# TianyiFranklinWang/MIRROR

Hardware: AMD Instinct MI355X
Metric: SSL samples/sec (slide+RNA pairs) (higher is better)
Workload: dtype bf16; 1 GPU; BASELINE c2: B=16/GPU x [4096 patch tokens x 1024-d] + [2048 genes], D=512, RNA depth 6 / 8 heads, train mode, local-batch InfoNCE; precision_policy=bf16, per_gpu_batch=16, global_batch=16, parallelism=dp1, grad_bucket_dtype=f32, step_launch=hip_graph

## Files before the change

mirror_amd/csrc/nystrom_fused.hip:

```cpp
#include <cstdlib>
#include <cstring>
#include "gemm_kernel.h"

namespace {

constexpr int NM = 256;
constexpr int ND = 64;
constexpr int NP = 72;
constexpr int NT = 256;
constexpr int TR = 128;

typedef __attribute__((address_space(3))) s16x4 lds_s16x4;
typedef short s16x8 __attribute__((ext_vector_type(8)));

__device__ __forceinline__ bf16x8 frag_kc(const bf16_t* img, int row0, int k0, int lane) {
    return *reinterpret_cast<const bf16x8*>(img + (row0 + (lane & 31)) * NP + k0 + 8 * (lane >> 5));
}
__device__ __forceinline__ bf16x8 frag_tr(const bf16_t* img, int col0, int kb, int lane) {
    const int g16 = lane >> 4, i = lane & 15, q = i >> 2, p = i & 3;
    const bf16_t* a0 = img + (kb + 4 * (g16 >> 1) + q) * NP + col0 + 16 * (g16 & 1) + 4 * p;
    s16x4 lo = __builtin_amdgcn_ds_read_tr16_b64_v4i16((lds_s16x4*)a0);
    s16x4 hi = __builtin_amdgcn_ds_read_tr16_b64_v4i16((lds_s16x4*)(a0 + 8 * NP));
    s16x8 v = __builtin_shufflevector(lo, hi, 0, 1, 2, 3, 4, 5, 6, 7);
    return __builtin_bit_cast(bf16x8, v);
}
__device__ __forceinline__ bf16x8 frag_g(const bf16_t* rowptr, int k0, int lane) {
    return *reinterpret_cast<const bf16x8*>(rowptr + k0 + 8 * (lane >> 5));
}
template <int T>
__device__ __forceinline__ bf16x8 pack8(const f32x16& a) {
    bf16x8 r;
#pragma unroll
    for (int j = 0; j < 8; j++) r[j] = (__bf16)a[8 * T + j];
    return r;
}
__device__ __forceinline__ f32x16 zero16() {
    f32x16 z;
#pragma unroll
    for (int r = 0; r < 16; r++) z[r] = 0.f;
    return z;
}
#define MFMA(a, b, c) __builtin_amdgcn_mfma_f32_32x32x16_bf16((a), (b), (c), 0, 0, 0)

constexpr float LOG2E = 1.4426950408889634f, LN2 = 0.6931471805599453f;
typedef float f32x8v __attribute__((ext_vector_type(8)));
typedef float f32x2v __attribute__((ext_vector_type(2)));
__device__ __forceinline__ float vsum16(const f32x16& a) {
    const f32x8v t8 = __builtin_shufflevector(a, a, 0, 1, 2, 3, 4, 5, 6, 7) + __builtin_shufflevector(a, a, 8, 9, 10, 11, 12, 13, 14, 15);
    const f32x4 t4 = __builtin_shufflevector(t8, t8, 0, 1, 2, 3) + __builtin_shufflevector(t8, t8, 4, 5, 6, 7);
    const f32x2v t2 = __builtin_shufflevector(t4, t4, 0, 1) + __builtin_shufflevector(t4, t4, 2, 3);
    return t2[0] + t2[1];
}
__device__ __forceinline__ float vmax16(const f32x16& a) {
    float m0 = fmaxf(fmaxf(a[0], a[1]), a[2]), m1 = fmaxf(fmaxf(a[3], a[4]), a[5]), m2 = fmaxf(fmaxf(a[6], a[7]), a[8]);
    float m3 = fmaxf(fmaxf(a[9], a[10]), a[11]), m4 = fmaxf(fmaxf(a[12], a[13]), a[14]);
    return fmaxf(fmaxf(fmaxf(m0, m1), fmaxf(m2, m3)), fmaxf(m4, a[15]));
}
__device__ __forceinline__ void exp2_16(f32x16& a) {
#pragma unroll
    for (int r = 0; r < 16; r++) a[r] = __builtin_amdgcn_exp2f(a[r]);
}
__device__ __forceinline__ f32x16 fma_splat(const f32x16& a, float m, float b) {
    const f32x2v mm = {m, m}, bb = {b, b};
    f32x16 r;
#pragma unroll
    for (int i = 0; i < 16; i += 2) {
        f32x2v x = {a[i], a[i + 1]};
        x = __builtin_elementwise_fma(x, mm, bb);
        r[i] = x[0];
        r[i + 1] = x[1];
    }
    return r;
}
constexpr float NEG_BIG = -1e30f;
__device__ __forceinline__ f32x16 rowvals16(const float* src, int hl) {
    f32x16 v;
#pragma unroll
    for (int gq = 0; gq < 4; gq++) {
        const f32x4 x = *reinterpret_cast<const f32x4*>(src + 8 * gq + 4 * hl);
        v[4 * gq] = x[0]; v[4 * gq + 1] = x[1]; v[4 * gq + 2] = x[2]; v[4 * gq + 3] = x[3];
    }
    return v;
}

template <int ROWS>
__device__ __forceinline__ void stage_rows(bf16_t* img, const bf16_t* __restrict__ src, long ld, int tid) {
#pragma unroll
    for (int i = 0; i < ROWS * 8 / NT; i++) {
        const int cid = tid + i * NT, r = cid >> 3, c = cid & 7;
        *reinterpret_cast<u32x4*>(img + r * NP + c * 8) = *reinterpret_cast<const u32x4*>(src + (long)r * ld + c * 8);
    }
}
template <int ROWS>
__device__ __forceinline__ void tile_load(u32x4 (&regs)[ROWS * 8 / NT], const bf16_t* __restrict__ src, long ld, int tid) {
#pragma unroll
    for (int i = 0; i < ROWS * 8 / NT; i++) {
        const int cid = tid + i * NT, r = cid >> 3, c = cid & 7;
        regs[i] = *reinterpret_cast<const u32x4*>(src + (long)r * ld + c * 8);
    }
}
template <int ROWS>
__device__ __forceinline__ void tile_store(const u32x4 (&regs)[ROWS * 8 / NT], bf16_t* img, int tid) {
#pragma unroll
    for (int i = 0; i < ROWS * 8 / NT; i++) {
        const int cid = tid + i * NT, r = cid >> 3, c = cid & 7;
// ... 323 lines not shown
    const int pr = tid >> 3, pc = tid & 7;
    u32x4 rq[NCH], rg[NCH], ro[NCH];
    float rl = 0.f;
    auto load_tiles = [&](int t) {
#pragma unroll
        for (int i = 0; i < NCH; i++) {
            const long row = (long)t * TR + pr + 64 * i;
            rq[i] = *reinterpret_cast<const u32x4*>(qb + row * 3 * D + pc * 8);
            rg[i] = *reinterpret_cast<const u32x4*>(gb + row * D + pc * 8);
            ro[i] = *reinterpret_cast<const u32x4*>(ob + row * D + pc * 8);
        }
        if (tid < TR) rl = lse1[(long)bh * g.n_p + (long)t * TR + tid];
    };
    load_tiles(t0);
#pragma unroll 1
    for (int t = t0; t < t1; t++) {
        __syncthreads();
#pragma unroll
        for (int i = 0; i < NCH; i++) {
            const int r = pr + 64 * i;
            *reinterpret_cast<u32x4*>(s_q + r * NP + pc * 8) = rq[i];
            *reinterpret_cast<u32x4*>(s_g + r * NP + pc * 8) = rg[i];
            float d = 0.f;
#pragma unroll
            for (int w = 0; w < 4; w++) {
                d += __uint_as_float(rg[i][w] << 16) * __uint_as_float(ro[i][w] << 16);
                d += __uint_as_float(rg[i][w] & 0xffff0000u) * __uint_as_float(ro[i][w] & 0xffff0000u);
            }
            d += __shfl_xor(d, 1, 64);
            d += __shfl_xor(d, 2, 64);
            d += __shfl_xor(d, 4, 64);
            if (pc == 0) {
                s_del[r] = -d * g.scale;
                delta1[(long)bh * g.n_p + (long)t * TR + r] = d;
            }
        }
        if (tid < TR) {
            s_lse[tid] = -rl * LOG2E;
            s_mr[tid] = masked ? g.mrow[(long)b * g.n_p + (long)t * TR + tid] : 1.f;
        }
        __syncthreads();
        if (t + 1 < t1) load_tiles(t + 1);
#pragma unroll
        for (int i = 0; i < 4; i++) {
            const f32x16 lv = rowvals16(s_lse + 32 * i, hl), dv = rowvals16(s_del + 32 * i, hl);
            f32x16 s = zero16(), dp = zero16();
#pragma unroll
            for (int ks = 0; ks < 4; ks++) {
                s = MFMA(frag_kc(s_q, 32 * i, 16 * ks, lane), klf[ks], s);
                dp = MFMA(frag_kc(s_g, 32 * i, 16 * ks, lane), w2f[ks], dp);
            }
            if (masked) {
                const f32x16 vr = rowvals16(s_mr + 32 * i, hl);
                s = s * g.scale2;
                mask_fill16(s, vr, ml);
                s = s + lv;
                exp2_16(s);
                dp = s * (dp * g.scale + dv);
                mask_zero16(dp, vr, ml);
            } else {
                s = s * g.scale2 + lv;
                exp2_16(s);
                dp = s * (dp * g.scale + dv);
            }
            const bf16x8 p0 = pack8<0>(s), p1 = pack8<1>(s), d0 = pack8<0>(dp), d1 = pack8<1>(dp);
#pragma unroll
            for (int nb = 0; nb < 2; nb++) {
                adw[nb] = MFMA(p0, frag_tr(s_g, 32 * nb, 32 * i, lane), adw[nb]);
                adw[nb] = MFMA(p1, frag_tr(s_g, 32 * nb, 32 * i + 16, lane), adw[nb]);
                adk[nb] = MFMA(d0, frag_tr(s_q, 32 * nb, 32 * i, lane), adk[nb]);
                adk[nb] = MFMA(d1, frag_tr(s_q, 32 * nb, 32 * i + 16, lane), adk[nb]);
            }
        }
    }
    float* dwb = dw2 + (long)bh * NM * ND;
    float* dkb = dlm + (long)b * NM * 2 * D + D + hd * ND;
#pragma unroll
    for (int nb = 0; nb < 2; nb++) {
        atomic_tile(dwb + (long)(32 * wave) * ND + 32 * nb, ND, adw[nb], hl, c);
        atomic_tile(dkb + (long)(32 * wave) * 2 * D + 32 * nb, 2 * D, adk[nb], hl, c);
    }
}

constexpr int A3_PART = NM * (ND + 2);
template <bool MASKED, bool RC = false>
__global__ __launch_bounds__(NT, 2) void nys_a3_fwd_kernel(const bf16_t* __restrict__ qkv, const bf16_t* __restrict__ lm,
                                                        float* __restrict__ av, float* __restrict__ lse3, float* __restrict__ part,
                                                        Geo g, int tiles_per_wg) {
    constexpr int VH = RC ? RC_HALO : 0;
    __shared__ __attribute__((aligned(16))) bf16_t s_k[TR * NP];
    __shared__ __attribute__((aligned(16))) bf16_t s_v_[(TR + 2 * VH) * NP];
    __shared__ __attribute__((aligned(16))) float s_mr[TR];
    bf16_t* const s_v = s_v_ + VH * NP;
    const int tid = threadIdx.x, lane = tid & 63, wave = tid >> 6, c = lane & 31, hl = lane >> 5;
    const int bh = blockIdx.y, b = bh / g.h, hd = bh % g.h, D = g.D;
    const long LD = g.lm_ld;
    const int t0 = blockIdx.x * tiles_per_wg, t1 = min(t0 + tiles_per_wg, g.n_p / TR);
    constexpr bool masked = MASKED;
    float ml[2] = {1.f, 1.f};
    if (masked) { ml[0] = g.mlm[(long)b * NM + 64 * wave + c]; ml[1] = g.mlm[(long)b * NM + 64 * wave + 32 + c]; }
    const bf16_t* qlb = lm + (long)b * NM * LD + hd * ND;
    bf16x8 qlf[2][4];
#pragma unroll
    for (int j = 0; j < 2; j++)
#pragma unroll
        for (int ks = 0; ks < 4; ks++) qlf[j][ks] = frag_g(qlb + (long)(64 * wave + 32 * j + c) * LD, 16 * ks, lane);
    const bf16_t* kb = qkv + (long)b * g.n_p * 3 * D + D + hd * ND;
    const bf16_t* vb = kb + D;
    float mrun[2] = {NEG_BIG, NEG_BIG}, lrun[2] = {0.f, 0.f};
    f32x16 o[2][2];
#pragma unroll
    for (int nb = 0; nb < 2; nb++)
#pragma unroll
        for (int j = 0; j < 2; j++) o[nb][j] = zero16();
    u32x4 rk[TR * 8 / NT], rv[TR * 8 / NT];
    tile_load<TR>(rk, kb + (long)t0 * TR * 3 * D, 3 * D, tid);
    tile_load<TR>(rv, vb + (long)t0 * TR * 3 * D, 3 * D, tid);
    u32x4 rh = {0u, 0u, 0u, 0u};
    const int hq = tid >> 3, hc = tid & 7, hrow = hq < RC_HALO ? hq - RC_HALO : TR + hq - RC_HALO;
    auto halo_load = [&](int t) {
        const long sr = (long)t * TR + hrow;
        rh = (u32x4){0u, 0u, 0u, 0u};
        if (sr >= 0 && sr < g.n_p) rh = *reinterpret_cast<const u32x4*>(vb + sr * 3 * D + hc * 8);
    };
    __shared__ __attribute__((aligned(16))) bf16x8 s_wf_[RC ? 4 * 64 : 1];
    if constexpr (RC) {
        halo_load(t0);
        if (wave == 0) {
            const float* wh = g.rc_w + hd * RC_TAPS;
#pragma unroll
            for (int ks = 0; ks < 4; ks++) {
                bf16x8 wv;
#pragma unroll
                for (int e = 0; e < 8; e++) {
                    const int k = 16 * ks + (e < 4 ? 4 * hl + e : 8 + 4 * hl + (e - 4));
                    const int jt = k - c;
                    const float x = wh[min(max(jt, 0), RC_TAPS - 1)];
                    wv[e] = (__bf16)((jt >= 0 && jt < RC_TAPS) ? x : 0.f);
                }
                s_wf_[ks * 64 + lane] = wv;
            }
        }
    }
#pragma unroll 1
    for (int t = t0; t < t1; t++) {
        __syncthreads();
        tile_store<TR>(rk, s_k, tid);
        tile_store<TR>(rv, s_v, tid);
        if constexpr (RC) *reinterpret_cast<u32x4*>(s_v + hrow * NP + hc * 8) = rh;
        if (tid < TR) s_mr[tid] = masked ? g.mrow[(long)b * g.n_p + (long)t * TR + tid] : 1.f;
        __syncthreads();
        if (t + 1 < t1) {
            tile_load<TR>(rk, kb + (long)(t + 1) * TR * 3 * D, 3 * D, tid);
            tile_load<TR>(rv, vb + (long)(t + 1) * TR * 3 * D, 3 * D, tid);
            if constexpr (RC) halo_load(t + 1);
        }
        if constexpr (RC) {
            bf16_t* orow = g.rc_out + ((long)b * g.n_p + (long)t * TR + 32 * wave + c) * D + hd * ND;
            int opq = 0;
            asm volatile("" : "+v"(opq));
            const bf16x8* s_wf = s_wf_ + opq;
#pragma unroll
            for (int nb = 0; nb < 2; nb++) {
                f32x16 a = zero16();
#pragma unroll
                for (int ks = 0; ks < 4; ks++) a = MFMA(frag_tr(s_v, 32 * nb, 32 * wave - RC_HALO + 16 * ks, lane), s_wf[ks * 64 + lane], a);
// ... 439 lines not shown
}

extern "C" int mh_nys_attn1_fwd(const void* qkv, const void* lm, const void* w2, void* out, float* lse1, const float* mrow,
                                const float* mlm, int B, int h, int n_p, int m, int dh, float scale, int accumulate, int64_t lm_ld, void* o1,
                                mh_stream s) {
    if (int e = check_geo("mh_nys_attn1_fwd", B, h, n_p, m, dh)) return e;
    MH_REQUIRE(lm_ld == 0 || (lm_ld >= 2L * h * ND && lm_ld % 8 == 0), "mh_nys_attn1_fwd: lm_ld must be 0 or a multiple of 8 >= 2 D");
    if (B == 0) return MH_OK;
    MH_REQUIRE((mrow == nullptr) == (mlm == nullptr), "mh_nys_attn1_fwd: mrow and mlm go together");
    const Geo g{h, n_p, h * ND, scale, scale * LOG2E, mrow, mlm, accumulate, lm_ld > 0 ? lm_ld : 2L * h * ND, nullptr, nullptr};
    MH_REQUIRE((((uintptr_t)o1) & 15) == 0, "mh_nys_attn1_fwd: o1 must be 16-byte aligned");
    NYS_LAUNCH(nys_a1_fwd_kernel, dim3(pick_walkers(B * h, n_p), B * h), dim3(NT), 0, (hipStream_t)s, (const bf16_t*)qkv, (const bf16_t*)lm,
                       (const bf16_t*)w2, (bf16_t*)out, lse1, g, Q8Out{}, (bf16_t*)o1);
    MH_LAUNCH_CHECK("mh_nys_attn1_fwd");
    return MH_OK;
}

extern "C" int mh_nys_attn1_fwd_q8(const void* qkv, const void* lm, const void* w2, void* out, float* lse1, int B, int h, int n_p, int m,
                                   int dh, float scale, int accumulate, void* q8, unsigned* ring, const float* tick, float margin,
                                   float* q8_scale, void* o1, mh_stream s) {
    if (int e = check_geo("mh_nys_attn1_fwd_q8", B, h, n_p, m, dh)) return e;
    if (B == 0) return MH_OK;
    MH_REQUIRE(q8 && ring && tick && q8_scale && margin >= 1.f && ((uintptr_t)q8 & 3) == 0, "mh_nys_attn1_fwd_q8: q8, ring, tick, scale and margin >= 1");
    const Geo g{h, n_p, h * ND, scale, scale * LOG2E, nullptr, nullptr, accumulate, 2L * h * ND, nullptr, nullptr};
    const Q8Out o{(unsigned char*)q8, ring, tick, margin, q8_scale};
    hipLaunchKernelGGL((nys_a1_fwd_kernel<false, true>), dim3(pick_walkers(B * h, n_p), B * h), dim3(NT), 0, (hipStream_t)s, (const bf16_t*)qkv,
                       (const bf16_t*)lm, (const bf16_t*)w2, (bf16_t*)out, lse1, g, o, (bf16_t*)o1);
    MH_LAUNCH_CHECK("mh_nys_attn1_fwd_q8");
    return MH_OK;
}

int pick_splits(int BH, int ntiles, int which);

extern "C" int64_t mh_nys_attn3_ws_floats(int B, int h, int n_p) {
    if (B <= 0 || h <= 0 || n_p < TR) return 0;
    const int splits = pick_splits(B * h, n_p / TR, 0);
    return splits > 1 ? (int64_t)B * h * splits * A3_PART : 0;
}

extern "C" int64_t mh_nys_attn3_workspace_bytes(int B, int h, int n_p) { return 4 * mh_nys_attn3_ws_floats(B, h, n_p); }

extern "C" int mh_nys_attn3_fwd(const void* qkv, const void* lm, float* av, float* lse3, float* workspace, int64_t ws_floats,
                                const float* mrow, const float* mlm, int B, int h, int n_p, int m, int dh, float scale, int64_t lm_ld,
                                const float* rc_w, void* rc_out, mh_stream s) {
    if (int e = check_geo("mh_nys_attn3_fwd", B, h, n_p, m, dh)) return e;
    MH_REQUIRE(lm_ld == 0 || (lm_ld >= 2L * h * ND && lm_ld % 8 == 0), "mh_nys_attn3_fwd: lm_ld must be 0 or a multiple of 8 >= 2 D");
    MH_REQUIRE((rc_w == nullptr) == (rc_out == nullptr) && (((uintptr_t)rc_out) & 15) == 0, "mh_nys_attn3_fwd: rc_w and rc_out (16-byte aligned) go together");
    if (B == 0) return MH_OK;
    const Geo g{h, n_p, h * ND, scale, scale * LOG2E, mrow, mlm, 0, lm_ld > 0 ? lm_ld : 2L * h * ND, rc_w, (bf16_t*)rc_out};
    const int ntiles = n_p / TR;
    int splits = pick_splits(B * h, ntiles, 0);
    if (!workspace || ws_floats < (int64_t)B * h * splits * A3_PART) splits = 1;
    const int tpw = (ntiles + splits - 1) / splits;
    splits = (ntiles + tpw - 1) / tpw;
    if (rc_w) {
        if (g.mrow) hipLaunchKernelGGL((nys_a3_fwd_kernel<true, true>), dim3(splits, B * h), dim3(NT), 0, (hipStream_t)s, (const bf16_t*)qkv,
                                       (const bf16_t*)lm, av, lse3, workspace, g, tpw);
        else hipLaunchKernelGGL((nys_a3_fwd_kernel<false, true>), dim3(splits, B * h), dim3(NT), 0, (hipStream_t)s, (const bf16_t*)qkv,
                                (const bf16_t*)lm, av, lse3, workspace, g, tpw);
    } else {
        NYS_LAUNCH(nys_a3_fwd_kernel, dim3(splits, B * h), dim3(NT), 0, (hipStream_t)s, (const bf16_t*)qkv, (const bf16_t*)lm, av,
                           lse3, workspace, g, tpw);
    }
    MH_LAUNCH_CHECK("mh_nys_attn3_fwd");
    if (splits > 1) {
        hipLaunchKernelGGL(nys_a3_combine_kernel, dim3(ND / 16, B * h), dim3(NM), 0, (hipStream_t)s, (const float*)workspace, av, lse3,
                           splits);
        MH_LAUNCH_CHECK("mh_nys_attn3_fwd(combine)");
    }
    return MH_OK;
}

int pick_splits(int BH, int ntiles, int which) {
    int splits = 1;
    while (BH * splits < 256 && splits * 2 <= ntiles) splits *= 2;
    return splits;
}

extern "C" int mh_nys_attn1_bwd(const void* qkv, const void* lm, const void* w2, const void* dout, const float* lse1, const void* o1,
                                float* delta1, void* dqkv, float* dw2, float* dlm, const float* mrow, const float* mlm, int B, int h,
                                int n_p, int m, int dh, float scale, int64_t lm_ld, int which, mh_stream s) {
    if (int e = check_geo("mh_nys_attn1_bwd", B, h, n_p, m, dh)) return e;
    MH_REQUIRE(lm_ld == 0 || (lm_ld >= 2L * h * ND && lm_ld % 8 == 0), "mh_nys_attn1_bwd: lm_ld must be 0 or a multiple of 8 >= 2 D");
    MH_REQUIRE(which >= 1 && which <= 3, "mh_nys_attn1_bwd: which = 1 (dw2, dk_l, delta1), 2 (dq from delta1) or 3 (both, in that order)");
    MH_REQUIRE(delta1 && (!(which & 1) || (o1 && dw2 && dlm && (((uintptr_t)o1) & 15) == 0)) && (!(which & 2) || dqkv),
               "mh_nys_attn1_bwd: missing buffer for the requested part");
    if (B == 0) return MH_OK;
    const Geo g{h, n_p, h * ND, scale, scale * LOG2E, mrow, mlm, 0, lm_ld > 0 ? lm_ld : 2L * h * ND, nullptr, nullptr};
    if (which & 1) {
        const int ntiles = n_p / TR, splits = pick_splits(B * h, ntiles, 1), tpw = (ntiles + splits - 1) / splits;
        NYS_LAUNCH(nys_a1_bwd_dw_kernel, dim3(splits, B * h), dim3(NTW), 0, (hipStream_t)s, (const bf16_t*)qkv,
                           (const bf16_t*)lm, (const bf16_t*)w2, (const bf16_t*)dout, lse1, (const bf16_t*)o1, delta1, dw2, dlm, g, tpw);
        MH_LAUNCH_CHECK("mh_nys_attn1_bwd(dw)");
    }
    if (which & 2) {
        NYS_LAUNCH(nys_a1_bwd_dq_kernel, dim3(pick_walkers(B * h, n_p), B * h), dim3(NT), 0, (hipStream_t)s, (const bf16_t*)qkv,
                           (const bf16_t*)lm, (const bf16_t*)w2, (const bf16_t*)dout, lse1, (const float*)delta1, (bf16_t*)dqkv, g);
        MH_LAUNCH_CHECK("mh_nys_attn1_bwd(dq)");
    }
    return MH_OK;
}

extern "C" int mh_nys_attn3_bwd(const void* qkv, const void* lm, const float* av, const void* dav, const float* lse3, float* delta3,
                                void* dqkv, float* dlm, const float* mrow, const float* mlm, int B, int h, int n_p, int m, int dh,
                                float scale, int64_t lm_ld, int one_pass, mh_stream s) {
    if (int e = check_geo("mh_nys_attn3_bwd", B, h, n_p, m, dh)) return e;
    MH_REQUIRE(lm_ld == 0 || (lm_ld >= 2L * h * ND && lm_ld % 8 == 0), "mh_nys_attn3_bwd: lm_ld must be 0 or a multiple of 8 >= 2 D");
    if (B == 0) return MH_OK;
    const Geo g{h, n_p, h * ND, scale, scale * LOG2E, mrow, mlm, 0, lm_ld > 0 ? lm_ld : 2L * h * ND, nullptr, nullptr};
    if (av) hipLaunchKernelGGL(nys_delta3_kernel, dim3(B * h), dim3(NM), 0, (hipStream_t)s, av, (const bf16_t*)dav, delta3);
    if (one_pass) {
        const int nsteps = n_p / HT;
        int splits = 1;
        while (B * h * splits < 256 && splits * 2 <= nsteps) splits *= 2;
        const int spw = (nsteps + splits - 1) / splits;
        NYS_LAUNCH(nys_a3_bwd_one_kernel, dim3((nsteps + spw - 1) / spw, B * h), dim3(NT8), 0, (hipStream_t)s, (const bf16_t*)qkv,
                           (const bf16_t*)lm, (const float*)delta3, (const bf16_t*)dav, lse3, (bf16_t*)dqkv, dlm, g, spw);
        MH_LAUNCH_CHECK("mh_nys_attn3_bwd(one pass)");
        return MH_OK;
    }
    NYS_LAUNCH(nys_a3_bwd_dkv_kernel, dim3(pick_walkers(B * h, n_p), B * h), dim3(NT), 0, (hipStream_t)s, (const bf16_t*)qkv,
                       (const bf16_t*)lm, (const float*)delta3, (const bf16_t*)dav, lse3, (bf16_t*)dqkv, g);
    MH_LAUNCH_CHECK("mh_nys_attn3_bwd(dkv)");
    const int ntiles = n_p / TR, splits = pick_splits(B * h, ntiles, 2), tpw = (ntiles + splits - 1) / splits;
    NYS_LAUNCH(nys_a3_bwd_dql_kernel, dim3(splits, B * h), dim3(NT), 0, (hipStream_t)s, (const bf16_t*)qkv,
                       (const bf16_t*)lm, (const float*)delta3, (const bf16_t*)dav, lse3, dlm, g, tpw);
    MH_LAUNCH_CHECK("mh_nys_attn3_bwd(dql)");
    return MH_OK;
}
```

mirror_amd/functional.py:

```python
from __future__ import annotations

from dataclasses import dataclass
from typing import List, Optional, Tuple

import os

import torch
from torch.autograd import Function

from . import kernels as K
from ._lib import ACT_NONE, ACT_RELU, MH_BF16, MH_F32

f32, bf16 = torch.float32, torch.bfloat16


@dataclass(frozen=True)
class Precision:
    name: str
    mma: int
    act: torch.dtype
    pinv_mma: int
    fp8_fwd: bool = False


# ... 1670 lines not shown
            av = K.gemm(a3, v, mma=mma, out_dtype=f32)
        pio = pm if (pm == MH_BF16 or A == f32) else mma
        w2 = None
        if side is not None and fused:
            w2 = torch.empty((Bn, h, m_l, dh), device=qkv.device, dtype=A)
            av_ready = torch.cuda.current_stream().record_event()
            with torch.cuda.stream(side):
                side.wait_event(av_ready)
                K.gemm(zf, av, out=w2, mma=pio)
        if fused and not rc_in_a3:
            K.resconv(qkv[..., 2 * D:], res_w.detach().contiguous(), out, h, transpose=False, accumulate=False)
        if side is not None:
            torch.cuda.current_stream().wait_stream(side)
            if chain:
                K.shared_chip = False
        if w2 is None:
            w2 = K.gemm(zf, av, mma=pio, out_dtype=A)
        o1 = None
        if fused:
            o1 = torch.empty_like(out)
            st8 = _fp8_state
            site = st8["sites"].get(q8_key) if (q8_key is not None and st8["tick"] is not None and kmask is None) else None
            if site is not None and st8["host_step"] - site[1] >= 2:
                q8 = torch.empty(out.shape, device=out.device, dtype=torch.uint8)
                lse1, sc8 = K.nys_attn1_fwd_q8(qkv, lm, w2, out, h, scale, True, q8, site[0], st8["tick"], o1=o1)
                q8_out.append((q8, sc8))
            else:
                lse1 = K.nys_attn1_fwd(qkv, lm, w2, out, h, scale, accumulate=True, kmask=kmask, o1=o1)
        else:
            K.gemm(a1, w2, out=_heads(out, 0, 1, h), mma=mma)
            K.resconv(qkv[..., 2 * D:], res_w.detach().contiguous(), out, h, transpose=False, accumulate=True)
        stats = (lse1, lse3) if fused else (a1, a3)
        ctx.has_o1 = o1 is not None
        ctx.save_for_backward(qkv, res_w, lm, stats[0], a2, stats[1], av, w2, st, zfT if chain else zf,
                              *([o1] if o1 is not None else []), *[t for it in saved for t in it])
        ctx.cfg = (heads, l, prec)
        ctx.chain = (chain, iters, fused)
        ctx.tile = tile
        ctx.kmask, ctx.link = kmask, link
        return out

    @staticmethod
    def backward(ctx, dout):
        qkv, res_w, lm, a1, a2, a3, av, w2, st, zf, *flat = ctx.saved_tensors
        o1 = None
        if ctx.has_o1:
            o1, flat = flat[0], flat[1:]
        chain, iters, fused = ctx.chain
        kmask = ctx.kmask
        if kmask is not None:
            mrow, mlm, lscale = kmask
        sm_bwd = (lambda y, dy, rm, cm: K.softmax_bwd(y, dy)) if kmask is None else K.softmax_masked_bwd
        zfT = zf if chain else None
        if chain:
            zf = zf.transpose(-1, -2)
        saved = None if chain else [tuple(flat[i:i + 4]) for i in range(0, len(flat), 4)]
        heads, l, prec = ctx.cfg
        A, mma, pm = prec.act, prec.mma, prec.pinv_mma
        Bn, n_p, D3 = qkv.shape
        D, h = D3 // 3, heads
        dh = D // h
        m = n_p // l
        scale = dh ** -0.5
        tr = lambda t: t.transpose(-1, -2)
        dout = dout.contiguous()
        if dout.dtype != A:
            dout = K.cast(dout, A)
        q, k, v = (_heads(qkv, i, 3, h) for i in range(3))
        ql, kl = _heads(lm, 0, 2, h), _heads(lm, 1, 2, h)
        dO = _heads(dout, 0, 1, h)
        de = dlm_out = None
        if ctx.lm_ext and A == bf16:
            de, dqkv, dlm_out = ext_rows_alloc(Bn, n_p, m, D3, 2 * D, qkv.device)
        else:
            dqkv = torch.empty_like(qkv)
        dq, dk, dv = (_heads(dqkv, i, 3, h) for i in range(3))
        rw = res_w.detach().contiguous()
        dres, dres_sunk = _gbuf(res_w, (rw.numel(),))
        if fused:
            lse1, lse3 = a1, a3
            dW2 = zeros((Bn, h, m, dh), qkv.device)
            dlm = zeros((Bn, m, 2 * D), qkv.device)
            delta1 = torch.empty_like(lse1)
            K.nys_attn1_bwd(qkv, lm, w2, dout, lse1, o1, delta1, dqkv, dW2, dlm, h, scale, kmask, which=1)
            if not (chain and _A1_DQ_IN_WINDOW):
                K.nys_attn1_bwd(qkv, lm, w2, dout, lse1, o1, delta1, dqkv, dW2, dlm, h, scale, kmask, which=2)
        else:
            dW2 = K.gemm(tr(a1), dO, mma=mma, out_dtype=f32)
            dlm = torch.empty((Bn, m, 2 * D), device=qkv.device, dtype=f32)
        dql, dkl = _heads(dlm, 0, 2, h), _heads(dlm, 1, 2, h)
        sd = f32 if pm == MH_F32 else bf16
        pio = pm if (pm == MH_BF16 or A == f32) else mma
        one2 = (chain and fused and A == bf16 and pio == MH_BF16 and dh == 64 and m == 256 and dW2.dtype == f32 and av.dtype == f32)
        dAV = dzb = None
        if one2:
            dzb, dAV = K.nys_dz_dav(dW2, av.contiguous(), zfT)
        else:
            dZ = K.gemm(dW2, tr(av), mma=pm, out_dtype=bf16 if (ctx.tile and _PINV_R32 and iters >= 1) else f32)
        side = dlm2 = None
        if chain:
            xb, chain_saved, z0 = flat
            work = K.pinv_chain_work_alloc(iters, Bn * h, m, qkv.device)
            dS2 = torch.empty_like(a2)
            dz0 = torch.empty_like(a2)
            if dzb is None:
                dzb = K.pinv_chain_pack(dZ)
            if fused and (kmask is None or _SIM2_MASKED):
                dlm2 = torch.empty_like(dlm)
            side = _side_stream(qkv.device)
            side.wait_stream(torch.cuda.current_stream())
            with torch.cuda.stream(side):
                K.pinv_chain_bwd(xb, chain_saved, dzb, work, dS2, dz0, iters)
                if (kmask is None or _SIM2_MASKED) and not ctx.z0_stored and a2.shape[-1] == 256:
                    K.pinv_s2_bwd(a2, dz0, st, dS2, _zeroed1(a2.device), mlm=mlm if kmask else None, heads=h)
                else:
                    K.pinv_z0_bwd(a2, z0 if ctx.z0_stored else None, dz0, st, dS2, _zeroed1(a2.device))
                    sm_bwd(a2, dS2, mlm if kmask else None, mlm if kmask else None)
                if dlm2 is not None:
                    K.gemm(tr(dS2), ql, out=_heads(dlm2, 1, 2, h), alpha=scale, mma=pio)
                    K.gemm(dS2, kl, out=_heads(dlm2, 0, 2, h), alpha=scale, mma=pio)
            K.shared_chip = True
        tile_side = ctx.tile and _TILE_SIDE and not chain
        if tile_side:
            dZ_ready = torch.cuda.current_stream().record_event()
            side = _side_stream(qkv.device)
            with torch.cuda.stream(side):
                side.wait_event(dZ_ready)
                dS2 = pinv_backward_tile(a2, saved, st, dZ, getattr(ctx, "a2b", None))
                sm_bwd(a2, dS2, mlm if kmask else None, mlm if kmask else None)
        if ctx.link is not None:
            ctx.link.run("wgrad")
        if fused and chain and _A1_DQ_IN_WINDOW:
            K.nys_attn1_bwd(qkv, lm, w2, dout, lse1, o1, delta1, dqkv, dW2, dlm, h, scale, kmask, which=2)
        rc_bwd_one = fused and _RC_FUSED and A == bf16
        if not rc_bwd_one:
            K.resconv_wgrad(qkv[..., 2 * D:], dout, dres, h)
        if dAV is None:
            dAV = K.gemm(tr(zf), dW2, mma=pio, out_dtype=A)
        if fused:
            K.nys_attn3_bwd(qkv, lm, av, dAV, lse3, dqkv, dlm, h, scale, kmask)
            if rc_bwd_one:
                K.resconv_bwd(dout, qkv[..., 2 * D:], rw, dqkv[..., 2 * D:], dres, h)
            else:
                K.resconv(dout, rw, dqkv[..., 2 * D:], h, transpose=True, accumulate=True)
        else:
            if (kmask is None and A == bf16 and mma == MH_BF16 and a1.dtype == bf16 and a1.is_contiguous()
                    and K.gemm_softmax_ok(n_p, m, dh, dO.dtype, w2.dtype)):
                dS1 = K.gemm(dO, tr(w2), mma=mma, out_dtype=bf16, softmax_bwd_of=a1)
            else:
                dS1 = K.gemm(dO, tr(w2), mma=mma, out_dtype=A)
                sm_bwd(a1, dS1, mrow if kmask else None, mlm if kmask else None)
            dS3 = K.gemm(dAV, tr(v), mma=mma, out_dtype=A)
            K.gemm(tr(a3), dAV, out=dv, mma=mma)
            K.resconv(dout, rw, dqkv[..., 2 * D:], h, transpose=True, accumulate=True)
            sm_bwd(a3, dS3, mlm if kmask else None, mrow if kmask else None)
            K.gemm(dS1, kl, out=dq, alpha=scale, mma=mma)
            K.gemm(tr(dS3), ql, out=dk, alpha=scale, mma=mma)
            K.gemm(tr(dS1), q, out=dkl, alpha=scale, mma=mma)
            K.gemm(dS3, k, out=dql, alpha=scale, mma=mma)
        if tile_side:
            torch.cuda.current_stream().wait_stream(side)
        elif side is not None:
            torch.cuda.current_stream().wait_stream(side)
            K.shared_chip = False
            del work
        else:
            dS2 = pinv_backward_tile(a2, saved, st, dZ, getattr(ctx, "a2b", None)) if ctx.tile else pinv_backward(a2, saved, st, dZ, pm, sd)
            sm_bwd(a2, dS2, mlm if kmask else None, mlm if kmask else None)
        if dlm2 is None:
# ... 615 lines not shown
```

mirror_amd/kernels.py:

```python
from __future__ import annotations

import ctypes as C
import os
from typing import Optional


import torch

from . import _lib
from ._lib import ACT_GELU, ACT_NONE, ACT_RELU, MH_BF16, MH_F32, GemmDesc, MirrorHipError

_DT = {torch.float32: MH_F32, torch.bfloat16: MH_BF16}


def dt(t: torch.Tensor) -> int:
    try:
        return _DT[t.dtype]
    except KeyError:
        raise MirrorHipError(f"unsupported dtype {t.dtype} (f32 / bf16 only)") from None


_raw_stream = getattr(torch._C, "_cuda_getCurrentRawStream", None)


# ... 937 lines not shown

def _lm_ld(lm: torch.Tensor) -> int:
    if lm.dim() != 3 or lm.stride(2) != 1 or lm.stride(0) != lm.shape[1] * lm.stride(1) or lm.stride(1) < lm.shape[2] or lm.stride(1) % 8:
        return 0
    return int(lm.stride(1))


def _nys_launch(name: str, flops: float, fn) -> None:
    if gemm_profiler is None:
        fn()
    else:
        gemm_profiler.launch_named(name, flops, fn)


def _nys_masks(kmask, B: int, n_p: int):
    if kmask is None:
        return None, None
    mrow, mlm = kmask[0], kmask[1]
    _chk(mrow, mlm)
    assert mrow.shape == (B, n_p) and mlm.shape == (B, NYS_FUSED_M) and mrow.dtype == mlm.dtype == torch.float32
    assert mrow.is_contiguous() and mlm.is_contiguous()
    return _p(mrow), _p(mlm)


def nys_attn1_fwd(qkv, lm, w2, out, heads: int, scale: float, accumulate: bool = False, kmask=None, o1=None) -> torch.Tensor:
    _chk(qkv, lm, w2, out, o1)
    B, n_p, _ = qkv.shape
    lse1 = torch.empty((B, heads, n_p), device=qkv.device, dtype=torch.float32)
    _nys_check("nys_attn1_fwd", B, heads, n_p, qkv=qkv, lm=lm, w2=w2, out=out, **({} if o1 is None else {"o1": o1}))
    _nys_launch("nys_a1_fwd_kernel", 2 * 2.0 * n_p * NYS_FUSED_M * NYS_FUSED_DH * B * heads,
                lambda: _lib.call("mh_nys_attn1_fwd", _p(qkv), _p(lm), _p(w2), _p(out), _p(lse1), *_nys_masks(kmask, B, n_p), B, heads,
                                  n_p, NYS_FUSED_M, NYS_FUSED_DH, scale, int(accumulate), _lm_ld(lm), _p(o1), stream=_stream()))
    return lse1


def nys_attn1_fwd_q8(qkv, lm, w2, out, heads: int, scale: float, accumulate: bool, q8, ring, tick, margin: float = 1.25, o1=None):
    _chk(qkv, lm, w2, out, q8, ring, tick)
    B, n_p, _ = qkv.shape
    if not (q8.dtype == torch.uint8 and q8.shape == out.shape and q8.is_contiguous() and ring.dtype == torch.int32 and ring.numel() == 3
            and tick.dtype == torch.float32):
        raise MirrorHipError("nys_attn1_fwd_q8: q8 uint8 shaped like out, int32[3] ring, f32 tick")
    lse1 = torch.empty((B, heads, n_p), device=qkv.device, dtype=torch.float32)
    sc = torch.empty((1,), device=qkv.device, dtype=torch.float32)
    _chk(o1)
    _nys_check("nys_attn1_fwd", B, heads, n_p, qkv=qkv, lm=lm.contiguous(), w2=w2, out=out, **({} if o1 is None else {"o1": o1}))
    lm = lm.contiguous()
    _nys_launch("nys_a1_fwd_kernel", 2 * 2.0 * n_p * NYS_FUSED_M * NYS_FUSED_DH * B * heads,
                lambda: _lib.call("mh_nys_attn1_fwd_q8", _p(qkv), _p(lm), _p(w2), _p(out), _p(lse1), B, heads, n_p, NYS_FUSED_M,
                                  NYS_FUSED_DH, scale, int(accumulate), _p(q8), _p(ring), _p(tick), float(margin), _p(sc), _p(o1),
                                  stream=_stream()))
    return lse1, sc


def nys_attn3_fwd(qkv, lm, heads: int, scale: float, kmask=None, rc=None):
    _chk(qkv, lm)
    B, n_p, _ = qkv.shape
    rc_w = rc_out = None
    if rc is not None:
        rc_w, rc_out = rc
        _chk(rc_w, rc_out)
        if (rc_w.dtype != torch.float32 or rc_w.numel() != heads * 33 or not rc_w.is_contiguous() or rc_out.dtype != torch.bfloat16
                or tuple(rc_out.shape) != (B, n_p, heads * NYS_FUSED_DH) or not rc_out.is_contiguous()):
            raise MirrorHipError("nys_attn3_fwd: rc = (f32 [h * 33] filters, contiguous bf16 [B, n_p, D] output)")
    av = torch.empty((B, heads, NYS_FUSED_M, NYS_FUSED_DH), device=qkv.device, dtype=torch.float32)
    lse3 = torch.empty((B, heads, NYS_FUSED_M), device=qkv.device, dtype=torch.float32)
    _nys_check("nys_attn3_fwd", B, heads, n_p, qkv=qkv, lm=lm)
    nws = int(_lib.load().mh_nys_attn3_ws_floats(B, heads, n_p))
    ws = torch.empty((nws,), device=qkv.device, dtype=torch.float32) if nws else None
    _nys_launch("nys_a3_fwd_kernel", 2 * 2.0 * n_p * NYS_FUSED_M * NYS_FUSED_DH * B * heads,
                lambda: _lib.call("mh_nys_attn3_fwd", _p(qkv), _p(lm), _p(av), _p(lse3), _p(ws), nws, *_nys_masks(kmask, B, n_p), B,
                                  heads, n_p, NYS_FUSED_M, NYS_FUSED_DH, scale, _lm_ld(lm), _p(rc_w), _p(rc_out), stream=_stream()))
    return av, lse3


def nys_attn1_bwd(qkv, lm, w2, dout, lse1, o1, delta1, dqkv, dw2, dlm, heads: int, scale: float, kmask=None, which: int = 3) -> None:
    _chk(qkv, lm, w2, dout, lse1, o1, delta1, dqkv, dw2, dlm)
    B, n_p, _ = qkv.shape
    ts = dict(qkv=qkv, lm=lm, w2=w2, dout=dout, lse1=lse1, delta1=delta1)
    if which & 1:
        ts.update(o1=o1, dw2=dw2, dlm=dlm)
    if which & 2:
        ts.update(dqkv=dqkv)
    _nys_check("nys_attn1_bwd", B, heads, n_p, **ts)
    prods = (4 if which & 1 else 0) + (3 if which & 2 else 0)
    _nys_launch("nys_a1_bwd_kernels", prods * 2.0 * n_p * NYS_FUSED_M * NYS_FUSED_DH * B * heads,
                lambda: _lib.call("mh_nys_attn1_bwd", _p(qkv), _p(lm), _p(w2), _p(dout), _p(lse1), _p(o1), _p(delta1), _p(dqkv),
                                  _p(dw2), _p(dlm), *_nys_masks(kmask, B, n_p), B, heads, n_p, NYS_FUSED_M, NYS_FUSED_DH, scale,
                                  _lm_ld(lm), int(which), stream=_stream()))


NYS_A3_BWD_ONE_PASS = True


def nys_attn3_bwd(qkv, lm, av, dav, lse3, dqkv, dlm, heads: int, scale: float, kmask=None, delta3=None, one_pass=None) -> None:
    one_pass = NYS_A3_BWD_ONE_PASS if one_pass is None else bool(one_pass)
    _chk(qkv, lm, av, dav, lse3, dqkv, dlm, delta3)
    B, n_p, _ = qkv.shape
    _nys_check("nys_attn3_bwd", B, heads, n_p, qkv=qkv, lm=lm, av=av, dav=dav, lse3=lse3, dqkv=dqkv, dlm=dlm)
    given = delta3 is not None
    if given and not (delta3.dtype == torch.float32 and delta3.is_contiguous() and delta3.numel() == lse3.numel()):
        raise MirrorHipError("nys_attn3_bwd: delta3 must be contiguous f32 [B, h, m]")
    if not given:
        delta3 = torch.empty_like(lse3)
    _nys_launch("nys_a3_bwd_kernels", 7 * 2.0 * n_p * NYS_FUSED_M * NYS_FUSED_DH * B * heads,
                lambda: _lib.call("mh_nys_attn3_bwd", _p(qkv), _p(lm), None if given else _p(av), _p(dav), _p(lse3), _p(delta3), _p(dqkv), _p(dlm),
                                  *_nys_masks(kmask, B, n_p), B, heads, n_p, NYS_FUSED_M, NYS_FUSED_DH, scale, _lm_ld(lm), int(one_pass),
                                  stream=_stream()))


def eye_minus(P: torch.Tensor, d: float) -> torch.Tensor:
    _chk(P)
    _contig(P, "eye_minus input")
    m = P.shape[-1]
    T = torch.empty_like(P)
    _lib.call("mh_eye_minus", _p(P), _p(T), d, P.numel() // (m * m), m, stream=_stream())
    return T


def seq_finish(seq: torch.Tensor, cls: torch.Tensor, N: int, add: int) -> None:
    _chk(seq, cls)
    B, n, D = seq.shape
    assert n == 1 + N + add and seq.is_contiguous() and cls.numel() == D and cls.dtype == torch.float32
    _lib.call("mh_seq_finish", _p(seq), _p(cls), B, N, add, D, dt(seq), stream=_stream())


def seq_finish_bwd(dseq: torch.Tensor, dcls: torch.Tensor, N: int, add: int) -> None:
    _chk(dseq, dcls)
    B, n, D = dseq.shape
    assert n == 1 + N + add and dseq.is_contiguous() and dcls.numel() == D and dcls.dtype == torch.float32
    _lib.call("mh_seq_finish_bwd", _p(dseq), _p(dcls), B, N, add, D, dt(dseq), stream=_stream())


def ppeg_merge(w7, w5, w3, b7, b5, b3):
    _chk(w7, w5, w3, b7, b5, b3)
    D = b7.numel()
    merged = torch.empty((49, D), device=w7.device, dtype=torch.float32)
    bsum = torch.empty((D,), device=w7.device, dtype=torch.float32)
    _lib.call("mh_ppeg_merge", _p(_contig(w7, "w7")), _p(_contig(w5, "w5")), _p(_contig(w3, "w3")), _p(b7), _p(b5), _p(b3),
              _p(merged), _p(bsum), D, stream=_stream())
    return merged, bsum


def ppeg(x: torch.Tensor, merged, bsum, S: int, flip: bool, out_dtype=None) -> torch.Tensor:
    _chk(x, merged, bsum)
    B, n, D = x.shape
    assert n == 1 + S * S and x.is_contiguous()
    y = torch.empty_like(x, dtype=out_dtype or x.dtype)
    _lib.call("mh_ppeg_fwd", _p(x), _p(y), _p(merged), _p(bsum), B, S, D, int(flip), dt(x), dt(y), stream=_stream())
    return y


def ppeg_wgrad(x, dout, dmerged, dbsum, S: int) -> None:
    _chk(x, dout, dmerged, dbsum)
    B, n, D = x.shape
    assert n == 1 + S * S and x.is_contiguous() and dout.is_contiguous() and dout.shape == x.shape
    _lib.call("mh_ppeg_wgrad", _p(x), _p(dout), _p(dmerged), _p(dbsum), B, S, D, dt(x), dt(dout), stream=_stream())


def ppeg_grad_scatter(dmerged, dbsum, dw7, dw5, dw3, db7, db5, db3) -> None:
    D = dbsum.numel()
    outs = (dw7, dw5, dw3, db7, db5, db3)
    _chk(dmerged, dbsum, *outs)
    for t, n in zip((dmerged,) + outs, (49 * D, 49 * D, 25 * D, 9 * D, D, D, D)):
        if t.dtype != torch.float32 or not t.is_contiguous() or t.numel() != n:
            raise MirrorHipError(f"ppeg_grad_scatter: expected a contiguous f32 tensor of {n} elements, got {tuple(t.shape)} {t.dtype}")
    _lib.call("mh_ppeg_grad_scatter", _p(dmerged), _p(dbsum), *[_p(t) for t in outs], D, stream=_stream())

# ... 688 lines not shown
```

Baseline: 2168 samples/s.

## Fuse Nystrom attention-1 backward dW/dK and dQ into one-pass kernel

Adds a single kernel that, per 128-row tile, computes the softmax probabilities and dS once, accumulates dW2 and dK_landmark, and writes dS to LDS so it can immediately compute dQ against the staged landmark keys. This replaces two launches that each recomputed the S and dP products, removing a recompute and a second pass over q, dout and o1. The cost is much larger LDS use (landmark keys plus a 256x136 dS buffer), which likely limits occupancy, and extra barriers per tile. It applies only when the dq part is not deferred into the chain window.

Result: faster. 2196 samples/s (median of 6 runs) (+1.3%).

```diff
diff --git a/mirror_amd/csrc/nystrom_fused.hip b/mirror_amd/csrc/nystrom_fused.hip
--- a/mirror_amd/csrc/nystrom_fused.hip
+++ b/mirror_amd/csrc/nystrom_fused.hip
@@ -16,11 +16,12 @@
 __device__ __forceinline__ bf16x8 frag_kc(const bf16_t* img, int row0, int k0, int lane) {
     return *reinterpret_cast<const bf16x8*>(img + (row0 + (lane & 31)) * NP + k0 + 8 * (lane >> 5));
 }
+template <int PITCH = NP>
 __device__ __forceinline__ bf16x8 frag_tr(const bf16_t* img, int col0, int kb, int lane) {
     const int g16 = lane >> 4, i = lane & 15, q = i >> 2, p = i & 3;
-    const bf16_t* a0 = img + (kb + 4 * (g16 >> 1) + q) * NP + col0 + 16 * (g16 & 1) + 4 * p;
+    const bf16_t* a0 = img + (kb + 4 * (g16 >> 1) + q) * PITCH + col0 + 16 * (g16 & 1) + 4 * p;
     s16x4 lo = __builtin_amdgcn_ds_read_tr16_b64_v4i16((lds_s16x4*)a0);
-    s16x4 hi = __builtin_amdgcn_ds_read_tr16_b64_v4i16((lds_s16x4*)(a0 + 8 * NP));
+    s16x4 hi = __builtin_amdgcn_ds_read_tr16_b64_v4i16((lds_s16x4*)(a0 + 8 * PITCH));
     s16x8 v = __builtin_shufflevector(lo, hi, 0, 1, 2, 3, 4, 5, 6, 7);
     return __builtin_bit_cast(bf16x8, v);
 }
@@ -510,6 +511,148 @@
     }
 }
 
+constexpr int DSP = TR + 8;
+template <bool MASKED>
+__global__ __launch_bounds__(NTW) void nys_a1_bwd_one_kernel(const bf16_t* __restrict__ qkv, const bf16_t* __restrict__ lm,
+                                                             const bf16_t* __restrict__ w2, const bf16_t* __restrict__ dout,
+                                                             const float* __restrict__ lse1, const bf16_t* __restrict__ o1,
+                                                             float* __restrict__ delta1, bf16_t* __restrict__ dqkv,
+                                                             float* __restrict__ dw2, float* __restrict__ dlm, Geo g,
+                                                             int tiles_per_wg) {
+    __shared__ __attribute__((aligned(16))) bf16_t s_kl[NM * NP];
+    __shared__ __attribute__((aligned(16))) bf16_t s_ds[NM * DSP];
+    __shared__ __attribute__((aligned(16))) bf16_t s_q[TR * NP];
+    __shared__ __attribute__((aligned(16))) bf16_t s_g[TR * NP];
+    __shared__ __attribute__((aligned(16))) float s_lse[TR];
+    __shared__ __attribute__((aligned(16))) float s_del[TR];
+    __shared__ __attribute__((aligned(16))) float s_mr[TR];
+    const int tid = threadIdx.x, lane = tid & 63, wave = tid >> 6, c = lane & 31, hl = lane >> 5;
+    const int bh = blockIdx.y, b = bh / g.h, hd = bh % g.h, D = g.D;
+    const long LD = g.lm_ld;
+    const int ntiles = g.n_p / TR;
+    const int t0 = blockIdx.x * tiles_per_wg, t1 = min(t0 + tiles_per_wg, ntiles);
+    if (t0 >= t1) return;
+    constexpr bool masked = MASKED;
+    const int lq = 32 * wave + c;
+    const float ml = masked ? g.mlm[(long)b * NM + lq] : 1.f;
+    const bf16_t* klb = lm + (long)b * NM * LD + D + hd * ND;
+    const bf16_t* w2b = w2 + (long)bh * NM * ND;
+#pragma unroll
+    for (int i = 0; i < NM * 8 / NTW; i++) {
+        const int cid = tid + i * NTW, r = cid >> 3, cc = cid & 7;
+        *reinterpret_cast<u32x4*>(s_kl + r * NP + cc * 8) = *reinterpret_cast<const u32x4*>(klb + (long)r * LD + cc * 8);
+    }
+    bf16x8 klf[4], w2f[4];
+#pragma unroll
+    for (int ks = 0; ks < 4; ks++) {
+        klf[ks] = frag_g(klb + (long)lq * LD, 16 * ks, lane);
+        w2f[ks] = frag_g(w2b + (long)lq * ND, 16 * ks, lane);
+    }
+    const bf16_t* qb = qkv + (long)b * g.n_p * 3 * D + hd * ND;
+    const bf16_t* gb = dout + (long)b * g.n_p * D + hd * ND;
+    const bf16_t* ob = o1 + (long)b * g.n_p * D + hd * ND;
+    f32x16 adw[2] = {zero16(), zero16()}, adk[2] = {zero16(), zero16()};
+    constexpr int NCH = TR * 8 / NTW;
+    const int pr = tid >> 3, pc = tid & 7;
+    u32x4 rq[NCH], rg[NCH], ro[NCH];
+    float rl = 0.f;
+    auto load_tiles = [&](int t) {
+#pragma unroll
+        for (int i = 0; i < NCH; i++) {
+            const long row = (long)t * TR + pr + 64 * i;
+            rq[i] = *reinterpret_cast<const u32x4*>(qb + row * 3 * D + pc * 8);
+            rg[i] = *reinterpret_cast<const u32x4*>(gb + row * D + pc * 8);
+            ro[i] = *reinterpret_cast<const u32x4*>(ob + row * D + pc * 8);
+        }
+        if (tid < TR) rl = lse1[(long)bh * g.n_p + (long)t * TR + tid];
+    };
+    auto stage_tiles = [&](int t) {
+#pragma unroll
+        for (int i = 0; i < NCH; i++) {
+            const int r = pr + 64 * i;
+            *reinterpret_cast<u32x4*>(s_q + r * NP + pc * 8) = rq[i];
+            *reinterpret_cast<u32x4*>(s_g + r * NP + pc * 8) = rg[i];
+            float d = 0.f;
+#pragma unroll
+            for (int w = 0; w < 4; w++) {
+                d += __uint_as_float(rg[i][w] << 16) * __uint_as_float(ro[i][w] << 16);
+                d += __uint_as_float(rg[i][w] & 0xffff0000u) * __uint_as_float(ro[i][w] & 0xffff0000u);
+            }
+            d += __shfl_xor(d, 1, 64);
+            d += __shfl_xor(d, 2, 64);
+            d += __shfl_xor(d, 4, 64);
+            if (pc == 0) {
+                s_del[r] = -d * g.scale;
+                delta1[(long)bh * g.n_p + (long)t * TR + r] = d;
+            }
+        }
+        if (tid < TR) {
+            s_lse[tid] = -rl * LOG2E;
+            s_mr[tid] = masked ? g.mrow[(long)b * g.n_p + (long)t * TR + tid] : 1.f;
+        }
+    };
+    load_tiles(t0);
+    stage_tiles(t0);
+    __syncthreads();
+    const int qb2 = wave & 3, dhalf = wave >> 2;
+#pragma unroll 1
+    for (int t = t0; t < t1; t++) {
+        const bool more = t + 1 < t1;
+        if (more) load_tiles(t + 1);
+#pragma unroll
+        for (int i = 0; i < 4; i++) {
+            const f32x16 lv = rowvals16(s_lse + 32 * i, hl), dv = rowvals16(s_del + 32 * i, hl);
+            f32x16 s = zero16(), dp = zero16();
+#pragma unroll
+            for (int ks = 0; ks < 4; ks++) {
+                s = MFMA(frag_kc(s_q, 32 * i, 16 * ks, lane), klf[ks], s);
+                dp = MFMA(frag_kc(s_g, 32 * i, 16 * ks, lane), w2f[ks], dp);
+            }
+            if (masked) {
+                const f32x16 vr = rowvals16(s_mr + 32 * i, hl);
+                s = s * g.scale2;
+                mask_fill16(s, vr, ml);
+                s = s + lv;
+                exp2_16(s);
+                dp = s * (dp * g.scale + dv);
+                mask_zero16(dp, vr, ml);
+            } else {
+                s = s * g.scale2 + lv;
+                exp2_16(s);
+                dp = s * (dp * g.scale + dv);
+            }
+            const bf16x8 p0 = pack8<0>(s), p1 = pack8<1>(s), d0 = pack8<0>(dp), d1 = pack8<1>(dp);
+#pragma unroll
+            for (int nb = 0; nb < 2; nb++) {
+                adw[nb] = MFMA(p0, frag_tr(s_g, 32 * nb, 32 * i, lane), adw[nb]);
+                adw[nb] = MFMA(p1, frag_tr(s_g, 32 * nb, 32 * i + 16, lane), adw[nb]);
+                adk[nb] = MFMA(d0, frag_tr(s_q, 32 * nb, 32 * i, lane), adk[nb]);
+                adk[nb] = MFMA(d1, frag_tr(s_q, 32 * nb, 32 * i + 16, lane), adk[nb]);
+            }
+            bf16_t* drow = s_ds + lq * DSP + 32 * i + 4 * hl;
+            const u32x4 dw0 = __builtin_bit_cast(u32x4, d0), dw1 = __builtin_bit_cast(u32x4, d1);
+            *reinterpret_cast<u32x2*>(drow) = u32x2{dw0[0], dw0[1]};
+            *reinterpret_cast<u32x2*>(drow + 8) = u32x2{dw0[2], dw0[3]};
+            *reinterpret_cast<u32x2*>(drow + 16) = u32x2{dw1[0], dw1[1]};
+            *reinterpret_cast<u32x2*>(drow + 24) = u32x2{dw1[2], dw1[3]};
+        }
+        __syncthreads();
+        if (more) stage_tiles(t + 1);
+        f32x16 a2 = zero16();
+#pragma unroll
+        for (int kt = 0; kt < NM / 16; kt++) a2 = MFMA(frag_tr(s_kl, 32 * dhalf, 16 * kt, lane), frag_tr<DSP>(s_ds, 32 * qb2, 16 * kt, lane), a2);
+        store_row8(dqkv + ((long)b * g.n_p + (long)t * TR + 32 * qb2 + c) * 3 * D + hd * ND + 32 * dhalf, a2, hl);
+        __syncthreads();
+    }
+    float* dwb = dw2 + (long)bh * NM * ND;
+    float* dkb = dlm + (long)b * NM * 2 * D + D + hd * ND;
+#pragma unroll
+    for (int nb = 0; nb < 2; nb++) {
+        atomic_tile(dwb + (long)(32 * wave) * ND + 32 * nb, ND, adw[nb], hl, c);
+        atomic_tile(dkb + (long)(32 * wave) * 2 * D + 32 * nb, 2 * D, adk[nb], hl, c);
+    }
+}
+
 constexpr int A3_PART = NM * (ND + 2);
 template <bool MASKED, bool RC = false>
 __global__ __launch_bounds__(NT, 2) void nys_a3_fwd_kernel(const bf16_t* __restrict__ qkv, const bf16_t* __restrict__ lm,
@@ -1115,11 +1258,18 @@
                                 int n_p, int m, int dh, float scale, int64_t lm_ld, int which, mh_stream s) {
     if (int e = check_geo("mh_nys_attn1_bwd", B, h, n_p, m, dh)) return e;
     MH_REQUIRE(lm_ld == 0 || (lm_ld >= 2L * h * ND && lm_ld % 8 == 0), "mh_nys_attn1_bwd: lm_ld must be 0 or a multiple of 8 >= 2 D");
-    MH_REQUIRE(which >= 1 && which <= 3, "mh_nys_attn1_bwd: which = 1 (dw2, dk_l, delta1), 2 (dq from delta1) or 3 (both, in that order)");
+    MH_REQUIRE(which >= 1 && which <= 3, "mh_nys_attn1_bwd: which = 1 (dw2, dk_l, delta1), 2 (dq from delta1) or 3 (all of them from the one-pass kernel)");
     MH_REQUIRE(delta1 && (!(which & 1) || (o1 && dw2 && dlm && (((uintptr_t)o1) & 15) == 0)) && (!(which & 2) || dqkv),
                "mh_nys_attn1_bwd: missing buffer for the requested part");
     if (B == 0) return MH_OK;
     const Geo g{h, n_p, h * ND, scale, scale * LOG2E, mrow, mlm, 0, lm_ld > 0 ? lm_ld : 2L * h * ND, nullptr, nullptr};
+    if (which == 3) {
+        const int ntiles = n_p / TR, splits = pick_splits(B * h, ntiles, 1), tpw = (ntiles + splits - 1) / splits;
+        NYS_LAUNCH(nys_a1_bwd_one_kernel, dim3(splits, B * h), dim3(NTW), 0, (hipStream_t)s, (const bf16_t*)qkv, (const bf16_t*)lm,
+                           (const bf16_t*)w2, (const bf16_t*)dout, lse1, (const bf16_t*)o1, delta1, (bf16_t*)dqkv, dw2, dlm, g, tpw);
+        MH_LAUNCH_CHECK("mh_nys_attn1_bwd(one pass)");
+        return MH_OK;
+    }
     if (which & 1) {
         const int ntiles = n_p / TR, splits = pick_splits(B * h, ntiles, 1), tpw = (ntiles + splits - 1) / splits;
         NYS_LAUNCH(nys_a1_bwd_dw_kernel, dim3(splits, B * h), dim3(NTW), 0, (hipStream_t)s, (const bf16_t*)qkv,
diff --git a/mirror_amd/functional.py b/mirror_amd/functional.py
--- a/mirror_amd/functional.py
+++ b/mirror_amd/functional.py
@@ -1776,9 +1776,8 @@
             dW2 = zeros((Bn, h, m, dh), qkv.device)
             dlm = zeros((Bn, m, 2 * D), qkv.device)
             delta1 = torch.empty_like(lse1)
-            K.nys_attn1_bwd(qkv, lm, w2, dout, lse1, o1, delta1, dqkv, dW2, dlm, h, scale, kmask, which=1)
-            if not (chain and _A1_DQ_IN_WINDOW):
-                K.nys_attn1_bwd(qkv, lm, w2, dout, lse1, o1, delta1, dqkv, dW2, dlm, h, scale, kmask, which=2)
+            K.nys_attn1_bwd(qkv, lm, w2, dout, lse1, o1, delta1, dqkv, dW2, dlm, h, scale, kmask,
+                            which=1 if (chain and _A1_DQ_IN_WINDOW) else 3)
         else:
             dW2 = K.gemm(tr(a1), dO, mma=mma, out_dtype=f32)
             dlm = torch.empty((Bn, m, 2 * D), device=qkv.device, dtype=f32)
diff --git a/mirror_amd/kernels.py b/mirror_amd/kernels.py
--- a/mirror_amd/kernels.py
+++ b/mirror_amd/kernels.py
@@ -1043,7 +1043,7 @@
     if which & 2:
         ts.update(dqkv=dqkv)
     _nys_check("nys_attn1_bwd", B, heads, n_p, **ts)
-    prods = (4 if which & 1 else 0) + (3 if which & 2 else 0)
+    prods = 5 if which == 3 else (4 if which & 1 else 0) + (3 if which & 2 else 0)
     _nys_launch("nys_a1_bwd_kernels", prods * 2.0 * n_p * NYS_FUSED_M * NYS_FUSED_DH * B * heads,
                 lambda: _lib.call("mh_nys_attn1_bwd", _p(qkv), _p(lm), _p(w2), _p(dout), _p(lse1), _p(o1), _p(delta1), _p(dqkv),
                                   _p(dw2), _p(dlm), *_nys_masks(kmask, B, n_p), B, heads, n_p, NYS_FUSED_M, NYS_FUSED_DH, scale,
```
